# lezhnev74/inverted_index_2

Hardware: NVIDIA B200
Metric: merged postings/s (higher is better)
Workload: dtype u32

## Files before the change

inverted_index_2_b200/csrc/k12_union.cu:

```cuda
#include <algorithm>
#include <cstdlib>
#include <vector>

#include "intcomp.cuh"
#include "keys.cuh"
#include "union.cuh"
#include "union_dev.cuh"

namespace ii2 {

constexpr int K1B_THREADS = 256;
constexpr int K1B_WARPS = K1B_THREADS / 32;
constexpr uint32_t CAP_I = 1024;
constexpr uint32_t K1B_HT = CAP_I > 512 ? 2048 : 1024;
static_assert(CAP_I % K1B_THREADS == 0 && CAP_I <= 1024 && CAP_I % 4 == 0,
              "tile = a whole number of instances per thread, 10-bit tile indexes");
constexpr uint32_t K1B_STAGE_CAP = CAP_I * 6;
constexpr uint32_t K1B_SMALL_D = 64;
constexpr uint32_t K1B_EMPTY = 0xFFFFFFFFu;
constexpr uint32_t K12_PENDING = 0xFFFFFFFFu;
constexpr uint32_t K1B_HEAVY = 0xFFFFFFFFu;

struct K1bArgs {
  const SegDesc* segs;
  int k;
  const uint32_t* part;
  const uint32_t* btb;
  const uint64_t* bpo;
  const uint64_t* bk_pos;
  const uint32_t* bk_cpl;
  const uint64_t* bk_P;
  GroupIn* gin;
  uint32_t* gath;
  uint64_t* src_ptr;
  uint32_t* src_len;
  uint32_t* bk_D;
  uint32_t bucket0;
  const uint32_t* list;
};


__device__ __noinline__ int k1b_tail_compare(const SegDesc* __restrict__ segs, int k, uint32_t ix,
                                             uint32_t nx, uint32_t iy, uint32_t ny, uint32_t skip) {
  int sx, sy;
  uint32_t tx, ty;
  locate_instance(segs, k, ix, sx, tx);
  locate_instance(segs, k, iy, sy, ty);
  const SegDesc& dx = segs[sx];
  const SegDesc& dy = segs[sy];
  const uint32_t ox = __ldg(dx.toff + tx);
  const uint32_t oy = __ldg(dy.toff + ty);
  for (uint32_t c = skip;; c += 16) {
    uint64_t hx, lx, hy, ly;
    load_key16(dx.tb, ox, nx, c, hx, lx);
    load_key16(dy.tb, oy, ny, c, hy, ly);
    if (hx != hy) return hx < hy ? -1 : 1;
    if (lx != ly) return lx < ly ? -1 : 1;
    if (!(nx > c + 16 && ny > c + 16)) break;
  }
  return nx < ny ? -1 : (nx > ny ? 1 : 0);
}

__host__ __device__ inline size_t k1b_smem_bytes(int k) {
  return (size_t)CAP_I * 24
         + (size_t)CAP_I * 4 * 3
         + (size_t)(4 * k) * 4 + (size_t)(2 * k + 2) * 4
         + (size_t)CAP_I * 2 * 2
         + (size_t)k * 40 + 16
         + (size_t)K1B_HT * 4 + 64;
}

constexpr int K1B_MIN_CTAS = 4;
template <bool LIST>
__global__ void __launch_bounds__(K1B_THREADS, K1B_MIN_CTAS) k1b_group_kernel(const K1bArgs a) {
  pdl_enter();
  extern __shared__ __align__(16) uint8_t smem_raw[];
  __shared__ uint64_t s_ws64[K1B_WARPS + 2];
  __shared__ uint32_t s_ws32[K1B_WARPS + 2];
  __shared__ uint32_t s_nreps, s_tot[2];

  const int k = a.k;
  uint8_t* sp = smem_raw;
  uint64_t* key_hi = reinterpret_cast<uint64_t*>(sp); sp += CAP_I * 8;
  uint64_t* key_lo = reinterpret_cast<uint64_t*>(sp); sp += CAP_I * 8;
  uint64_t* key_x = reinterpret_cast<uint64_t*>(sp); sp += CAP_I * 8;
  uint32_t* cg = reinterpret_cast<uint32_t*>(sp); sp += CAP_I * 4;
  uint32_t* inst_a = reinterpret_cast<uint32_t*>(sp); sp += CAP_I * 4;
  uint32_t* pbase = reinterpret_cast<uint32_t*>(sp); sp += CAP_I * 4;
  uint16_t* tlen = reinterpret_cast<uint16_t*>(sp); sp += CAP_I * 2;
  uint16_t* reps = reinterpret_cast<uint16_t*>(sp); sp += CAP_I * 2;
  sp += (16 - (reinterpret_cast<uintptr_t>(sp) & 15)) & 15;
  uint32_t* table = reinterpret_cast<uint32_t*>(sp); sp += K1B_HT * 4;
  uint32_t* cur = reinterpret_cast<uint32_t*>(sp); sp += k * 4;
  uint32_t* mm = reinterpret_cast<uint32_t*>(sp); sp += k * 4;
  uint32_t* hib = reinterpret_cast<uint32_t*>(sp); sp += k * 4;
  uint32_t* endr = reinterpret_cast<uint32_t*>(sp); sp += k * 4;
  uint32_t* rstart = reinterpret_cast<uint32_t*>(sp);
  sp += (2 * k + 2) * 4;
  sp += (8 - (reinterpret_cast<uintptr_t>(sp) & 7)) & 7;
  const uint8_t** sg_tb = reinterpret_cast<const uint8_t**>(sp); sp += k * 8;
  const uint32_t** sg_toff = reinterpret_cast<const uint32_t**>(sp); sp += k * 8;
  const uint64_t** sg_poff = reinterpret_cast<const uint64_t**>(sp); sp += k * 8;
  const uint32_t** sg_post = reinterpret_cast<const uint32_t**>(sp); sp += k * 8;
  uint32_t* sg_bl = reinterpret_cast<uint32_t*>(sp);
  uint32_t* sbase = table;
  uint32_t kp2 = 1;
  while (kp2 < (uint32_t)k) kp2 <<= 1;

  const uint32_t tid = threadIdx.x;
  const unsigned lane = lane_id(), warp = warp_id();
  const uint32_t b = LIST ? a.list[blockIdx.x] : a.bucket0 + blockIdx.x;
  uint32_t W = (uint32_t)(a.bk_pos[b + 1] - a.bk_pos[b]);
  if (W == 0) {
    if (tid == 0) a.bk_D[b] = 0;
    return;
  }
  {
    const uint32_t r0 = b, r1 = b + 1;
    for (int s = tid; s < k; s += K1B_THREADS) {
      cur[s] = a.part[(uint64_t)r0 * k + s];
      endr[s] = a.part[(uint64_t)r1 * k + s];
      const SegDesc sd = a.segs[s];
      sg_tb[s] = sd.tb;
      sg_toff[s] = sd.toff;
      sg_poff[s] = sd.poff;
      sg_post[s] = sd.post;
      sg_bl[s] = sd.base - sd.lo;
      asm volatile("prefetch.global.L2 [%0];" ::"l"(sd.toff + cur[s]));
      asm volatile("prefetch.global.L2 [%0];" ::"l"(sd.poff + cur[s]));
      if (endr[s] - cur[s] > 12) asm volatile("prefetch.global.L2 [%0];" ::"l"(sd.poff + endr[s]));
    }
  }
  const uint64_t rec_base = a.bk_pos[b];
  const uint32_t cpl = a.bk_cpl[b];
  uint32_t* const gath = a.gath + a.bk_P[b];
  uint32_t dcount = 0;
  uint32_t icount = 0;
  uint32_t pcount = 0;
  uint32_t ecount = 0;
  __syncthreads();

  while (W > 0) {
    uint32_t size;
    const uint32_t* mmp;
    if (W <= CAP_I) {
      mmp = endr;
      size = W;
    } else {
      mmp = mm;
      for (int s = tid; s < k; s += K1B_THREADS) hib[s] = endr[s];
      __syncthreads();
      for (;;) {
        uint64_t best = 0;
        for (int s = tid; s < k; s += K1B_THREADS) {
          const uint64_t cand = ((uint64_t)(hib[s] - cur[s]) << 32) | (uint32_t)s;
          best = cand > best ? cand : best;
        }
#pragma unroll
        for (int d = 16; d > 0; d >>= 1) {
          const uint64_t o = __shfl_xor_sync(0xffffffffu, best, d);
          best = o > best ? o : best;
        }
        __syncthreads();
        if (lane == 0) s_ws64[warp] = best;
        __syncthreads();
        for (int w2 = 0; w2 < K1B_WARPS; w2++) best = s_ws64[w2] > best ? s_ws64[w2] : best;
        const int spv = (int)(uint32_t)best;
        const uint32_t win = (uint32_t)(best >> 32);
        const uint32_t mid = cur[spv] + (win >> 1);
        const KeyedTerm pivot = keyed_term(a.segs[spv], mid);
        uint32_t part_sum = 0;
        for (int s = tid; s < k; s += K1B_THREADS) {
          const uint32_t m = s == spv ? mid : keyed_lower_bound(a.segs[s], cur[s], hib[s], pivot);
          mm[s] = m;
          part_sum += m - cur[s];
        }
        uint32_t tot;
        block_exclusive_scan(part_sum, s_ws32, tot);
        size = tot;
        if (size <= CAP_I) break;
        for (int s = tid; s < k; s += K1B_THREADS) hib[s] = mm[s];
        __syncthreads();
      }
      __syncthreads();
    }

    if (k <= 128 && warp != 0) {
    } else if (k <= 128) {
      uint32_t v[4], sum = 0;
#pragma unroll
      for (int j = 0; j < 4; j++) {
        const int s = lane * 4 + j;
        v[j] = s < k ? mmp[s] - cur[s] : 0u;
        sum += v[j];
      }
      uint32_t ex = warp_inclusive_scan(sum) - sum;
#pragma unroll
      for (int j = 0; j < 4; j++) {
        const int s = lane * 4 + j;
        if (s < k) rstart[s] = ex;
        ex += v[j];
      }
      for (uint32_t s2 = k + lane; s2 <= kp2; s2 += 32) rstart[s2] = size;
    } else {
      uint32_t run = 0;
      for (int base = 0; base < k; base += K1B_THREADS) {
        const int s = base + tid;
        const uint32_t v = s < k ? mmp[s] - cur[s] : 0u;
        uint32_t tot;
        const uint32_t ex = block_exclusive_scan(v, s_ws32, tot);
        if (s < k) rstart[s] = run + ex;
        run += tot;
      }
      for (uint32_t s2 = k + tid; s2 <= kp2; s2 += K1B_THREADS) rstart[s2] = size;
    }
    for (uint32_t i = tid; i < K1B_HT / 4; i += K1B_THREADS)
      reinterpret_cast<uint4*>(table)[i] = make_uint4(~0u, ~0u, ~0u, ~0u);
    for (uint32_t i = 4 * tid; i < CAP_I; i += 4 * K1B_THREADS)
      *reinterpret_cast<uint4*>(cg + i) = make_uint4(0u, 0u, 0u, 0u);
    if (tid == 0) s_nreps = 0;
    __syncthreads();

    auto tail_compare = [&](uint32_t x, uint32_t y) -> int {
      const uint32_t skip = cpl + 24;
      const uint32_t nx = tlen[x], ny = tlen[y];
      if (nx > skip && ny > skip)
        return k1b_tail_compare(a.segs, k, inst_a[x], nx, inst_a[y], ny, skip);
      return nx < ny ? -1 : (nx > ny ? 1 : 0);
    };
    auto less = [&](uint16_t x, uint16_t y) -> bool {
      const uint64_t hx = key_hi[x], hy = key_hi[y];
      if (hx != hy) return hx < hy;
      const uint64_t lx = key_lo[x], ly = key_lo[y];
      if (lx != ly) return lx < ly;
      const uint64_t xx = key_x[x], xy = key_x[y];
      if (xx != xy) return xx < xy;
      return tail_compare(x, y) < 0;
    };

    constexpr int PER = CAP_I / K1B_THREADS;
    uint64_t pp[PER];
    uint32_t pl[PER];
    uint32_t og[PER];
    {
      int sg[PER];
      uint32_t ix[PER], to[PER], tn[PER];
      uint64_t p1[PER];
#pragma unroll
      for (int j = 0; j < PER; j++) {
        const uint32_t i = tid + j * K1B_THREADS;
        sg[j] = -1;
        if (i < size) {
          uint32_t lo = 0;
          for (uint32_t step = kp2 >> 1; step > 0; step >>= 1)
            if (rstart[lo + step] <= i) lo += step;
          sg[j] = (int)lo;
          ix[j] = cur[lo] + (i - rstart[lo]);
        }
      }
#pragma unroll
      for (int j = 0; j < PER; j++) {
        if (sg[j] >= 0) {
          const uint32_t* const toff_s = sg_toff[sg[j]];
          const uint64_t* const poff_s = sg_poff[sg[j]];
          to[j] = __ldg(toff_s + ix[j]);
          tn[j] = __ldg(toff_s + ix[j] + 1);
          pp[j] = __ldg(poff_s + ix[j]);
          p1[j] = __ldg(poff_s + ix[j] + 1);
        }
      }
#pragma unroll
      for (int j = 0; j < PER; j++)
        if (sg[j] >= 0) asm volatile("prefetch.global.L2 [%0];" ::"l"(sg_tb[sg[j]] + to[j] + cpl));
#pragma unroll
      for (int j = 0; j < PER; j++) {
        if (sg[j] >= 0) {
          const uint32_t i = tid + j * K1B_THREADS;
          const uint32_t n = tn[j] - to[j];
          uint64_t kh, kl;
          const uint8_t* const tb_s = sg_tb[sg[j]];
          const uint32_t* const post_s = sg_post[sg[j]];
          const uint32_t inst_s = sg_bl[sg[j]] + ix[j];
          load_key16(tb_s, to[j], n, cpl, kh, kl);
          key_hi[i] = kh;
          key_lo[i] = kl;
          key_x[i] = load_key_x(tb_s, to[j], n, cpl);
          tlen[i] = (uint16_t)n;
          inst_a[i] = inst_s;
          pl[j] = (p1[j] - pp[j]) > 0xFFFFFFFEull ? 0xFFFFFFFFu : (uint32_t)(p1[j] - pp[j]);
          pp[j] = reinterpret_cast<uint64_t>(post_s + pp[j]);
          asm volatile("prefetch.global.L2 [%0];" ::"l"(pp[j]));
        }
      }
    }
    __threadfence_block();

#pragma unroll
    for (int j = 0; j < PER; j++) {
      const uint32_t i = tid + j * K1B_THREADS;
      if (i >= size) break;
      const uint64_t kh = key_hi[i], kl = key_lo[i];
      uint32_t h = (uint32_t)kh * 0x9E3779B1u ^ (uint32_t)(kh >> 32) * 0x85EBCA77u ^
                   (uint32_t)kl * 0xC2B2AE3Du ^ (uint32_t)(kl >> 32) * 0x27D4EB2Fu;
      h = (h ^ (h >> 15)) * 0x2C1B3C6Du + tlen[i];
      uint32_t slot = (h ^ (h >> 13)) & (K1B_HT - 1);
      uint32_t rep;
      for (;;) {
        const uint32_t prev = atomicCAS(&table[slot], K1B_EMPTY, i);
        if (prev == K1B_EMPTY) {
          rep = i;
          reps[atomicAdd(&s_nreps, 1u)] = (uint16_t)i;
          break;
        }
        if (*(volatile uint64_t*)&key_hi[prev] == kh && *(volatile uint64_t*)&key_lo[prev] == kl &&
            *(volatile uint16_t*)&tlen[prev] == tlen[i] &&
            *(volatile uint64_t*)&key_x[prev] == key_x[i] && tail_compare(i, prev) == 0) {
          rep = prev;
          break;
        }
        slot = (slot + 1) & (K1B_HT - 1);
      }
      og[j] = (rep << 20) |
              (atomicAdd(&cg[rep], (1u << 20) | (pl[j] > REG_CAP ? REG_CAP + 1 : pl[j])) & 0xFFFFFu);
    }
    __syncthreads();
    const uint32_t D = s_nreps;

    if (D <= K1B_SMALL_D) {
      const unsigned sub = lane & 7u;
#pragma unroll 1
      for (uint32_t t0 = warp * 4; t0 < D; t0 += K1B_WARPS * 4) {
        const uint32_t t = t0 + (lane >> 3);
        const bool valid = t < D;
        const uint32_t me = valid ? reps[t] : 0u;
        uint32_t rank = 0, ib = 0, pst = 0, est = 0;
        if (valid) {
          const uint64_t mh = key_hi[me], ml = key_lo[me], mx = key_x[me];
#pragma unroll 1
          for (uint32_t j = sub; j < D; j += 8) {
            const uint32_t o = reps[j];
            const uint64_t oh = key_hi[o];
            bool lt = oh < mh;
            if (oh == mh && o != me) {
              const uint64_t ol = key_lo[o], ox = key_x[o];
              lt = ol != ml ? ol < ml : (ox != mx ? ox < mx : tail_compare(o, me) < 0);
            }
            const uint32_t c = cg[o];
            const uint32_t len = c & 0xFFFFFu;
            const bool lg = lt && len <= REG_CAP;
            rank += lt ? 1u : 0u;
            ib += lt ? c >> 20 : 0u;
            pst += lg ? len : 0u;
            est += lg ? enc_slot_words(len) : 0u;
          }
        }
#pragma unroll
        for (int d = 4; d > 0; d >>= 1) {
          rank += __shfl_xor_sync(0xffffffffu, rank, d);
          ib += __shfl_xor_sync(0xffffffffu, ib, d);
          pst += __shfl_xor_sync(0xffffffffu, pst, d);
          est += __shfl_xor_sync(0xffffffffu, est, d);
        }
        if (valid && sub == 0) {
          const uint32_t cme = cg[me];
          const uint32_t len = cme & 0xFFFFFu;
          const bool light = len <= REG_CAP;
          const uint32_t src = (uint32_t)rec_base + icount + ib;
          uint4* rec = reinterpret_cast<uint4*>(a.gin + rec_base + dcount + rank);
          rec[0] = make_uint4(inst_a[me], tlen[me], src, cme >> 20);
          rec[1] = make_uint4(len, pcount + pst, ecount + est, 0u);
          sbase[me] = src;
          pbase[me] = light ? pcount + pst : K1B_HEAVY;
          if (rank == D - 1) {
            s_tot[0] = pst + (light ? len : 0u);
            s_tot[1] = est + (light ? enc_slot_words(len) : 0u);
          }
        }
      }
    } else {
      bitonic_sort_any(reps, D, tid, (uint32_t)K1B_THREADS, less, [] { __syncthreads(); });
      __syncthreads();
      uint32_t run_i = 0, run_p = 0, run_e = 0;
      for (uint32_t base = 0; base < D; base += K1B_THREADS) {
        const uint32_t r = base + tid;
        uint32_t me = 0, ci = 0, li = 0, ei = 0;
        uint32_t len = 0;
        if (r < D) {
          me = reps[r];
          ci = cg[me] >> 20;
          len = cg[me] & 0xFFFFFu;
          if (len <= REG_CAP) {
            li = len;
            ei = enc_slot_words(li);
          }
        }
        uint32_t ti, tp, te;
        const uint32_t xi = block_exclusive_scan(ci, s_ws32, ti);
        const uint32_t xp = block_exclusive_scan(li, s_ws32, tp);
        const uint32_t xe = block_exclusive_scan(ei, s_ws32, te);
        if (r < D) {
          GroupIn g;
          g.inst = inst_a[me];
          g.tlen = tlen[me];
          g.src = (uint32_t)rec_base + icount + run_i + xi;
          g.c = ci;
          g.L = len;
          g.pst = pcount + run_p + xp;
          g.eslot = ecount + run_e + xe;
          g.pad = 0;
          a.gin[rec_base + dcount + r] = g;
          sbase[me] = g.src;
          pbase[me] = len <= REG_CAP ? g.pst : K1B_HEAVY;
        }
        run_i += ti;
        run_p += tp;
        run_e += te;
      }
      if (tid == 0) {
        s_tot[0] = run_p;
        s_tot[1] = run_e;
      }
    }
    __syncthreads();

    const uint32_t tile_p = s_tot[0];
    const bool staged = tile_p <= K1B_STAGE_CAP;
    uint32_t* const stage = reinterpret_cast<uint32_t*>(key_hi);
    auto copy_source = [](const uint32_t* __restrict__ src, uint32_t* __restrict__ dst, uint32_t n) {
      uint32_t t = 0;
#pragma unroll 1
      for (; t + 4 <= n; t += 4) {
        const uint32_t x0 = __ldg(src + t), x1 = __ldg(src + t + 1), x2 = __ldg(src + t + 2),
                       x3 = __ldg(src + t + 3);
        dst[t] = x0;
        dst[t + 1] = x1;
        dst[t + 2] = x2;
        dst[t + 3] = x3;
      }
      if (t < n) {
        const uint32_t x0 = __ldg(src + t);
        const uint32_t x1 = t + 1 < n ? __ldg(src + t + 1) : 0u;
        const uint32_t x2 = t + 2 < n ? __ldg(src + t + 2) : 0u;
        dst[t] = x0;
        if (t + 1 < n) dst[t + 1] = x1;
        if (t + 2 < n) dst[t + 2] = x2;
      }
    };
#pragma unroll
    for (int j = 0; j < PER; j++) {
      const uint32_t i = tid + j * K1B_THREADS;
      if (i < size) {
        const uint32_t g = og[j] >> 20;
        const uint32_t pb = pbase[g];
        if (pb != K1B_HEAVY) {
          const uint32_t* src = reinterpret_cast<const uint32_t*>(pp[j]);
          const uint32_t at = pb + (og[j] & 0xFFFFFu);
          if (staged)
            copy_source(src, stage + (at - pcount), pl[j]);
          else
            copy_source(src, gath + at, pl[j]);
        } else {
          const uint32_t at = sbase[g] + ((atomicSub(&cg[g], 1u << 20) >> 20) - 1u);
          a.src_ptr[at] = pp[j];
          a.src_len[at] = pl[j];
        }
      }
    }
    if (staged) {
      __syncthreads();
      uint32_t* const out = gath + pcount;
      const uint32_t head = min(tile_p, (uint32_t)((16u - ((uintptr_t)out & 15u)) & 15u) >> 2);
      if (tid < head) out[tid] = stage[tid];
      const uint32_t nvec = (tile_p - head) >> 2;
      for (uint32_t v = tid; v < nvec; v += K1B_THREADS) {
        const uint32_t e = head + 4 * v;
        *reinterpret_cast<uint4*>(out + e) =
            make_uint4(stage[e], stage[e + 1], stage[e + 2], stage[e + 3]);
      }
      const uint32_t tail0 = head + 4 * nvec;
      if (tail0 + tid < tile_p) out[tail0 + tid] = stage[tail0 + tid];
    }
    dcount += D;
    icount += size;
    pcount += s_tot[0];
    ecount += s_tot[1];
    W -= size;
    if (W == 0) break;
    __syncthreads();
    for (int s = tid; s < k; s += K1B_THREADS) cur[s] = mmp[s];
    __syncthreads();
  }
  if (tid == 0) a.bk_D[b] = dcount;
}


constexpr int K2B_THREADS = 128;
constexpr int K2B_WARPS = K2B_THREADS / 32;
constexpr uint32_t K2B_HALF = 128;
constexpr uint32_t K2B_ENC_WORDS = 3 + 2 * 129 + 1 + (5 * 127 + 3) / 4 + 1;
constexpr uint32_t K2B_EBUF = (K2B_ENC_WORDS + 7) & ~7u;
static_assert(K2B_EBUF / 2 >= 1 + (5 * 127 + 3) / 4, "var-byte stream of 127 values fits a half");

struct K2bArgs {
  const uint64_t* bk_pos;
  const uint64_t* bk_P;
  const uint64_t* bk_E;
  const uint32_t* bk_D;
  const GroupIn* gin;
  RemovedSet rem;
  int want_enc, want_dec, keep_empty;
  GroupRec* recs;
  uint32_t* gath;
  uint32_t* tmp_enc;
  uint64_t* bk_raw;
  uint32_t nb1;
  uint32_t* n_large;
  uint32_t* large_rec;
  uint32_t* large_bucket;
  uint32_t bucket0;
  const uint32_t* list;
};

constexpr int K2B_MIN_CTAS = 8;
template <bool LIST>
__global__ void __launch_bounds__(K2B_THREADS, K2B_MIN_CTAS) k2b_union_kernel(const K2bArgs a) {
  pdl_enter();
  __shared__ __align__(16) uint32_t s_buf[K2B_WARPS][REG_CAP];
  __shared__ __align__(16) uint32_t s_enc[K2B_WARPS][K2B_EBUF];
  const unsigned lane = lane_id(), warp = warp_id();
  const unsigned half = lane >> 4, hl = lane & 15u;
  const uint32_t b = LIST ? a.list[blockIdx.x] : a.bucket0 + blockIdx.x;
  const uint32_t D = a.bk_D[b];
  if (D == 0) return;
  const uint64_t rec_base = a.bk_pos[b];
  uint32_t* const gath = a.gath + a.bk_P[b];
  uint32_t* const enc_base = a.tmp_enc + a.bk_E[b];
  uint32_t acc_t = 0, acc_tb = 0, acc_e = 0;
  uint64_t acc_p = 0;
  const GroupIn g_none = {0u, 0u, 0u, 0u, 0u, 0u, 0u, 0u};
  GroupIn g_next = g_none;
  if (2 * warp + half < D) g_next = a.gin[rec_base + 2 * warp + half];
#pragma unroll 1
  for (uint32_t p0 = 2 * warp; p0 < D; p0 += 2 * K2B_WARPS) {
    const uint32_t r = p0 + half;
    const bool has = r < D;
    const GroupIn g = g_next;
    {
      const uint32_t rn = r + 2 * K2B_WARPS;
      g_next = g_none;
      if (rn < D) g_next = a.gin[rec_base + rn];
    }

    const bool heavy = has && g.L > REG_CAP;
    const bool wide = has && !heavy && g.L >= K2B_HALF;
    if (heavy && hl == 0) {
      const uint32_t slot = atomicAdd(a.n_large, 1u);
      a.large_rec[slot] = (uint32_t)(rec_base + r);
      a.large_bucket[slot] = b;
      GroupRec rec;
      rec.inst = g.inst;
      rec.tlen = g.tlen;
      rec.dec = 0;
      rec.eoff = 0;
      rec.enc = 0;
      rec.cnt = K12_PENDING;
      a.recs[rec_base + r] = rec;
    }
    {
      const bool mine = has && !heavy && !wide;
      const uint32_t L = mine ? g.L : 0u;
      uint32_t* const slot = gath + g.pst;
      uint32_t* const buf = s_buf[warp] + half * K2B_HALF;
      uint32_t* const ebuf = s_enc[warp] + half * (K2B_EBUF / 2);
      const uint32_t outn = union_blocked<16>(slot, buf, L, g.c > 1, a.rem);
      if (a.want_dec)
        for (uint32_t e = hl; e < outn; e += 16) slot[e] = buf[e];
      uint32_t enc = 0;
      uint32_t* const enc_dst = enc_base + g.eslot;
      if (a.want_enc) {
        enc = encode_small_blocked<16>(buf, outn, ebuf);
        for (uint32_t e = hl; e < enc; e += 16) enc_dst[e] = ebuf[e];
      }
      if (mine && hl == 0) {
        GroupRec rec;
        rec.inst = g.inst;
        rec.tlen = g.tlen;
        rec.dec = reinterpret_cast<uint64_t>(slot);
        rec.eoff = a.want_enc ? reinterpret_cast<uint64_t>(enc_dst) : 0ull;
        rec.cnt = outn;
        rec.enc = enc;
        a.recs[rec_base + r] = rec;
        if (outn || a.keep_empty) {
          acc_t += 1;
          acc_tb += g.tlen;
          acc_p += outn;
          acc_e += enc;
        }
      }
      __syncwarp();
    }
    unsigned wmask = __ballot_sync(0xffffffffu, wide && hl == 0);
    while (wmask) {
      const int src = __ffs(wmask) - 1;
      wmask &= wmask - 1;
      GroupIn w;
      w.inst = __shfl_sync(0xffffffffu, g.inst, src);
      w.tlen = __shfl_sync(0xffffffffu, g.tlen, src);
      w.c = __shfl_sync(0xffffffffu, g.c, src);
      w.L = __shfl_sync(0xffffffffu, g.L, src);
      w.pst = __shfl_sync(0xffffffffu, g.pst, src);
      w.eslot = __shfl_sync(0xffffffffu, g.eslot, src);
      const uint32_t rw = p0 + (src >> 4);
      uint32_t* const slot = gath + w.pst;
      uint32_t* const buf = s_buf[warp];
      uint32_t* const ebuf = s_enc[warp];
      const uint32_t outn = union_blocked<32>(slot, buf, w.L, w.c > 1, a.rem);
      if (a.want_dec)
        for (uint32_t e = lane; e < outn; e += 32) slot[e] = buf[e];
      uint32_t enc = 0;
      uint32_t* const enc_dst = enc_base + w.eslot;
      if (a.want_enc && outn) {
        enc = encode_shared_warp(buf, outn, ebuf);
        for (uint32_t e = lane; e < enc; e += 32) enc_dst[e] = ebuf[e];
      }
      if (lane == 0) {
        GroupRec rec;
        rec.inst = w.inst;
        rec.tlen = w.tlen;
        rec.dec = reinterpret_cast<uint64_t>(slot);
        rec.eoff = a.want_enc ? reinterpret_cast<uint64_t>(enc_dst) : 0ull;
        rec.cnt = outn;
        rec.enc = enc;
        a.recs[rec_base + rw] = rec;
        if (outn || a.keep_empty) {
          acc_t += 1;
          acc_tb += w.tlen;
          acc_p += outn;
          acc_e += enc;
        }
      }
      __syncwarp();
    }
  }
  if (hl == 0 && acc_t) {
    unsigned long long* bo = reinterpret_cast<unsigned long long*>(a.bk_raw);
    atomicAdd(&bo[0ull * a.nb1 + b], (unsigned long long)acc_t);
    atomicAdd(&bo[1ull * a.nb1 + b], (unsigned long long)acc_tb);
    atomicAdd(&bo[2ull * a.nb1 + b], (unsigned long long)acc_p);
    atomicAdd(&bo[3ull * a.nb1 + b], (unsigned long long)acc_e);
  }
}

constexpr uint32_t MW_CAP = 1024;
constexpr int MW_V = 32;
constexpr int MW_WARPS = 4;
constexpr int MW_MIN_CTAS = 5;
constexpr uint32_t MW_BUF = MW_CAP + MW_CAP / 32 + 8;
constexpr uint32_t MW_EBUF = 3 + 8 * 129 + 1 + 1 + 6;
static_assert(MW_EBUF >= kMaxSegs + 1, "source prefix fits the stream buffer");

struct MwArgs {
  const uint32_t* n_in_list;
  const uint32_t* in_rec;
  const uint32_t* in_bucket;
  const GroupIn* gin;
  const uint64_t* src_ptr;
  const uint32_t* src_len;
  GroupRec* recs;
  RemovedSet rem;
  int want_enc, keep_empty;
  uint64_t* bk_raw;
  uint32_t nb1;
  uint32_t* cursor;
  uint32_t* n_out_list;
  uint32_t* out_rec;
  uint32_t* out_bucket;
  uint32_t* out_post;
  uint32_t* out_enc;
  unsigned long long* out_cursor;
};

__global__ void __launch_bounds__(MW_WARPS * 32, MW_MIN_CTAS) k2_mwarp_kernel(const MwArgs a) {
  pdl_enter();
  __shared__ __align__(16) uint32_t s_buf[MW_WARPS][MW_BUF];
  __shared__ __align__(16) uint32_t s_enc[MW_WARPS][MW_EBUF];
  const unsigned lane = lane_id(), warp = warp_id();
  uint32_t* const buf = s_buf[warp];
  uint32_t* const ebuf = s_enc[warp];
  uint32_t* const moff = ebuf;
  for (;;) {
    uint32_t item = 0;
    if (lane == 0) item = atomicAdd(a.cursor, 1u);
    item = __shfl_sync(0xffffffffu, item, 0);
    if (item >= *a.n_in_list) return;
    const uint32_t rec = a.in_rec[item], bucket = a.in_bucket[item];
    const GroupIn g = a.gin[rec];
    const uint32_t c = g.c, beg = g.src;
    uint32_t run = 0;
    for (uint32_t base = 0; base < c; base += 32) {
      const uint32_t i = base + lane;
      uint32_t li = i < c ? a.src_len[beg + i] : 0u;
      li = li > MW_CAP + 1 ? MW_CAP + 1 : li;
      const uint32_t inc = warp_inclusive_scan(li);
      if (i < c) moff[i] = min(run + inc - li, MW_CAP + 1);
      run = min(run + __shfl_sync(0xffffffffu, inc, 31), MW_CAP + 1);
    }
    if (run > MW_CAP) {
      if (lane == 0) {
        const uint32_t at = atomicAdd(a.n_out_list, 1u);
        a.out_rec[at] = rec;
        a.out_bucket[at] = bucket;
      }
// ... 699 lines not shown
    const uint32_t ny = std::min<uint32_t>(32768, h_nl - y0);
    uint64_t maxL = 0;
    for (uint32_t i = 0; i < ny; i++) maxL = std::max(maxL, lens[y0 + i]);
    LargeArgs b2 = la;
    b2.rec += y0;
    if (b2.presorted) b2.presorted += y0;
    if (b2.bucket) b2.bucket += y0;
    b2.len += y0;
    b2.off += y0;
    b2.eoff += y0;
    const unsigned gx = (unsigned)std::max<uint64_t>(1, std::min<uint64_t>((maxL + 4095) / 4096, 2048));
    dim3 grid(gx, ny);
    k2_large_gather<<<grid, 256, 0, s>>>(b2, nullptr, 0);
    II2_LAUNCHED();
    uint64_t maxS = 0;
    for (uint32_t i = 0; i < ny; i++) {
      const uint32_t g = y0 + i;
      if (!h_pre[g]) {
        maxS = std::max(maxS, lens[g]);
        continue;
      }
      const uint64_t words = ((uint64_t)h_max[g] >> 5) + 1;
      const uint64_t n_chunks = (words + BM_CHUNK_WORDS - 1) / BM_CHUNK_WORDS;
      II2_CUDA_TRY(cudaMemsetAsync(bm_words.p, 0, words * 4, s));
      k2_large_gather<<<(unsigned)std::min<uint64_t>((lens[g] + 255) / 256, 148 * 16), 256, 0, s>>>(
          b2, bm_words.p, i);
      II2_LAUNCHED();
      k2_bm_count<<<div_up((n_chunks + 1) * 32, 256), 256, 0, s>>>(bm_words.p, words, n_chunks,
                                                                   bm_counts.p, la.rem);
      II2_LAUNCHED();
      II2_TRY(exclusive_scan_u64(bm_counts.p, n_chunks + 1, nullptr, s));
      k2_bm_expand<<<div_up(n_chunks * 32, 256), 256, 0, s>>>(bm_words.p, words, n_chunks,
                                                              bm_counts.p, la.tmp + offs[g],
                                                              d_len.p + g);
      II2_LAUNCHED();
    }
    maxL = maxS;
    k2_large_tile_sort<<<grid, 512, 0, s>>>(b2);
    II2_LAUNCHED();
    for (uint64_t kk = 2ull * LG_TILE; (kk >> 1) < maxL; kk <<= 1) {
      k2_large_stage<<<grid, 256, 0, s>>>(b2, kk, 0);
      II2_LAUNCHED();
      for (uint64_t j = kk >> 2; j >= LG_TILE; j >>= 1) {
        k2_large_stage<<<grid, 256, 0, s>>>(b2, kk, j);
        II2_LAUNCHED();
      }
      k2_large_tile_merge<<<grid, 512, 0, s>>>(b2, kk);
      II2_LAUNCHED();
    }
    k2_large_finish<<<ny, 1024, 0, s>>>(b2);
    II2_LAUNCHED();
  }
  II2_CUDA_TRY(cudaStreamSynchronize(s));
  return II2_OK;
}

static bool k12_takes_fused(uint64_t N, int k) {
  const char* fused_env = getenv("II2_FUSED");
  const bool fused_on = fused_env ? atoi(fused_env) != 0 : N <= 65536;
  return fused_on && k12f_supported(k);
}

int k12_union(const MergePlan& plan, const RemovedSet& rem, bool want_dec, bool want_enc,
              bool keep_empty, uint64_t n_in, uint64_t tb_in, UnionOut& u, cudaStream_t s) {
  u.keep_empty = keep_empty;
  u.want_dec = want_dec;
  u.want_enc = want_enc;
  const uint32_t B = plan.n_buckets, N = plan.n_total;
  const int k = plan.k;
  u.fused = k12_takes_fused(N, k);
  DevBuf<GroupIn> gin;
  DevBuf<uint64_t> src_ptr;
  DevBuf<uint32_t> src_len;
  II2_TRY(gin.alloc_scratch(N, s));
  II2_TRY(src_ptr.alloc_scratch(N, s));
  II2_TRY(src_len.alloc_scratch(N, s));
  II2_TRY(u.recs.alloc_scratch(N, s));
  II2_TRY(u.bk_D.alloc_scratch(B, s));
  II2_TRY(u.bk_raw.alloc_scratch(4 * (size_t)(B + 1), s));
  II2_TRY(u.bk_out.alloc_scratch(4 * (size_t)(B + 1), s));
  II2_TRY(u.totals.alloc_scratch(8, s));
  const uint64_t enc_cap = n_in + n_in / 4 + 6ull * N + 64;
  if (want_enc) II2_TRY(u.tmp_enc.alloc_scratch(enc_cap, s, 16));
  II2_TRY(u.tmp_post.alloc_scratch(n_in, s, 16));
  const uint32_t large_cap = (uint32_t)std::min<uint64_t>(N, n_in / REG_CAP + 1);
  DevBuf<uint32_t> large_u32;
  II2_TRY(large_u32.alloc_scratch(8 * (size_t)large_cap, s));
  DevBuf<unsigned long long> med_cursor;
  II2_TRY(med_cursor.alloc_scratch(8, s));
  II2_CUDA_TRY(cudaMemsetAsync(med_cursor.p, 0, 64, s));
  II2_TRY(u.med_post.alloc_scratch(n_in, s, 16));
  if (want_enc) II2_TRY(u.med_enc.alloc_scratch(n_in + n_in / 4 + 16ull * large_cap + 64, s, 16));
  II2_CUDA_TRY(cudaMemsetAsync(u.totals.p, 0, 64, s));
  II2_CUDA_TRY(cudaMemsetAsync(u.bk_raw.p, 0, 4 * (size_t)(B + 1) * 8, s));
  II2_TRY(u.bk_mode.alloc_scratch(B, s));
  if (u.fused) {
    II2_TRY(u.st_tb.alloc_scratch(tb_in, s, 64));
    II2_TRY(u.st_off.alloc_scratch(3 * (size_t)N, s));
    II2_TRY(u.def_list.alloc_scratch(B, s));
  } else {
    II2_CUDA_TRY(cudaMemsetAsync(u.bk_mode.p, 0, (size_t)B * 4, s));
  }

  K1bArgs a1;
  a1.segs = plan.segs;
  a1.k = k;
  a1.part = plan.part.p;
  a1.btb = plan.btb.p;
  a1.bpo = plan.bpo.p;
  a1.bk_pos = plan.bk_pos();
  a1.bk_cpl = plan.bk_cpl.p;
  a1.bk_P = plan.bk_P();
  a1.gin = gin.p;
  a1.gath = u.tmp_post.p;
  a1.src_ptr = src_ptr.p;
  a1.src_len = src_len.p;
  a1.bk_D = u.bk_D.p;
  K2bArgs a2;
  a2.bk_pos = plan.bk_pos();
  a2.bk_P = plan.bk_P();
  a2.bk_E = plan.bk_E();
  a2.bk_D = u.bk_D.p;
  a2.gin = gin.p;
  a2.rem = rem;
  a2.want_enc = want_enc ? 1 : 0;
  a2.want_dec = want_dec ? 1 : 0;
  a2.keep_empty = keep_empty ? 1 : 0;
  a2.recs = u.recs.p;
  a2.gath = u.tmp_post.p;
  a2.tmp_enc = u.tmp_enc.p;
  a2.bk_raw = u.bk_raw.p;
  a2.nb1 = B + 1;
  a2.n_large = reinterpret_cast<uint32_t*>(u.totals.p + 6);
  a2.large_rec = large_u32.p;
  a2.large_bucket = large_u32.p + large_cap;
  const size_t smem = k1b_smem_bytes(k);
  static size_t attr = 0;
  if (smem > attr) {
    const size_t want = std::max(k1b_smem_bytes(kMaxSegs), smem);
    II2_CUDA_TRY(cudaFuncSetAttribute(k1b_group_kernel<false>, cudaFuncAttributeMaxDynamicSharedMemorySize,
                                      (int)want));
    II2_CUDA_TRY(cudaFuncSetAttribute(k1b_group_kernel<true>, cudaFuncAttributeMaxDynamicSharedMemorySize,
                                      (int)want));
    attr = want;
  }
  auto general = [&](uint32_t grid, const uint32_t* list) -> int {
    a1.bucket0 = a2.bucket0 = 0;
    a1.list = a2.list = list;
    {
      ProfScope scope("k1b_group", s);
      if (list) {
        II2_LAUNCH_CHAIN(k1b_group_kernel<true>, grid, K1B_THREADS, smem, s, a1);
      } else {
        II2_LAUNCH_CHAIN(k1b_group_kernel<false>, grid, K1B_THREADS, smem, s, a1);
      }
    }
    {
      ProfScope scope("k2b_union", s);
      if (list) {
        II2_LAUNCH_CHAIN(k2b_union_kernel<true>, grid, K2B_THREADS, 0, s, a2);
      } else {
        II2_LAUNCH_CHAIN(k2b_union_kernel<false>, grid, K2B_THREADS, 0, s, a2);
      }
    }
    {
      ProfScope scope("k2_medium", s);
      uint32_t* const mid_rec = large_u32.p + 4 * (size_t)large_cap;
      uint32_t* const mid_bucket = large_u32.p + 5 * (size_t)large_cap;
      uint32_t* const n_mid = reinterpret_cast<uint32_t*>(med_cursor.p + 3);
      MwArgs w2;
      w2.n_in_list = a2.n_large;
      w2.in_rec = a2.large_rec;
      w2.in_bucket = a2.large_bucket;
      w2.gin = gin.p;
      w2.src_ptr = src_ptr.p;
      w2.src_len = src_len.p;
      w2.recs = u.recs.p;
      w2.rem = rem;
      w2.want_enc = want_enc ? 1 : 0;
      w2.keep_empty = keep_empty ? 1 : 0;
      w2.bk_raw = u.bk_raw.p;
      w2.nb1 = B + 1;
      w2.cursor = reinterpret_cast<uint32_t*>(med_cursor.p + 2) + 1;
      w2.n_out_list = n_mid;
      w2.out_rec = mid_rec;
      w2.out_bucket = mid_bucket;
      w2.out_post = u.med_post.p;
      w2.out_enc = u.med_enc.p;
      w2.out_cursor = med_cursor.p;
      II2_LAUNCH_CHAIN(k2_mwarp_kernel, kNumSMs * MW_MIN_CTAS, MW_WARPS * 32, 0, s, w2);
      uint32_t* const mid2_rec = large_u32.p + 6 * (size_t)large_cap;
      uint32_t* const mid2_bucket = large_u32.p + 7 * (size_t)large_cap;
      uint32_t* const n_mid2 = reinterpret_cast<uint32_t*>(med_cursor.p + 3) + 1;
      MedArgs m;
      m.n_large = n_mid;
      m.large_rec = mid_rec;
      m.large_bucket = mid_bucket;
      m.gin = gin.p;
      m.src_ptr = src_ptr.p;
      m.src_len = src_len.p;
      m.recs = u.recs.p;
      m.rem = rem;
      m.want_enc = want_enc ? 1 : 0;
      m.keep_empty = keep_empty ? 1 : 0;
      m.bk_raw = u.bk_raw.p;
      m.nb1 = B + 1;
      m.cursor = reinterpret_cast<uint32_t*>(med_cursor.p + 4);
      m.n_huge = n_mid2;
      m.huge_rec = mid2_rec;
      m.huge_bucket = mid2_bucket;
      m.out_post = u.med_post.p;
      m.out_enc = u.med_enc.p;
// ... 92 lines not shown
```

inverted_index_2_b200/csrc/union.cuh:

```cuda
#pragma once
#include "plan.cuh"

namespace ii2 {

struct GroupRec {
  uint64_t dec;
  uint64_t eoff;
  uint32_t inst;
  uint32_t tlen;
  uint32_t cnt;
  uint32_t enc;
};

struct __align__(16) GroupIn {
  uint32_t inst;
  uint32_t tlen;
  uint32_t src;
  uint32_t c;
  uint32_t L;
  uint32_t pst;
  uint32_t eslot;
  uint32_t pad;
};


struct LargeArgs {
  const uint32_t* rec;
  const uint32_t* bucket;
  const GroupIn* gin;
  const uint64_t* src_ptr;
  const uint32_t* src_len;
  uint64_t* len;
  const uint64_t* off;
  const uint64_t* eoff;
  uint32_t* tmp;
  uint32_t* enc;
  GroupRec* recs;
  RemovedSet rem;
  int want_enc, keep_empty;
  int always_sort;
  const uint8_t* presorted;
  uint64_t* bk_raw;
  uint32_t nb1;
};

constexpr uint32_t F_MAXK = 256;
constexpr uint32_t K12F_RECORDS = 0;
constexpr uint32_t K12F_DENSE = 1;
constexpr uint32_t K12F_DEFERRED = 2;

struct K12fArgs {
  const SegDesc* segs;
  int k;
  const uint32_t* part;
  const uint32_t* btb;
  const uint64_t* bpo;
  const uint64_t* bk_pos;
  const uint32_t* bk_cpl;
  const uint64_t* bk_P;
  const uint64_t* bk_E;
  const uint64_t* bk_TB;
  RemovedSet rem;
  int want_enc, want_dec, keep_empty;
  uint32_t* bk_D;
  uint32_t* bk_mode;
  uint64_t* bk_raw;
  uint32_t nb1;
  uint8_t* st_tb;
  uint32_t* st_toff;
  uint32_t* st_eoff;
  uint32_t* st_poff;
  uint32_t* st_enc;
  uint32_t* st_post;
  uint32_t* n_def;
  uint32_t* def_list;
};
bool k12f_supported(int k);
int k12f_launch(const K12fArgs& a, uint32_t n_buckets, cudaStream_t s);

int k2_large_run(LargeArgs la, uint32_t n_groups, DevBuf<uint32_t>& large_tmp,
                 DevBuf<uint32_t>& large_enc, cudaStream_t s);

struct UnionOut {
  DevBuf<GroupRec> recs;
  DevBuf<uint32_t> tmp_post;
  DevBuf<uint32_t> tmp_enc;
  DevBuf<uint32_t> large_enc;
  DevBuf<uint32_t> large_tmp;
  DevBuf<uint32_t> med_post;
  DevBuf<uint32_t> med_enc;
  DevBuf<uint32_t> bk_D;
  bool fused = false;
  DevBuf<uint8_t> st_tb;
  DevBuf<uint32_t> st_off;
  DevBuf<uint32_t> bk_mode;
  DevBuf<uint32_t> def_list;
  uint32_t n_def = 0;
  DevBuf<uint64_t> bk_raw;
  DevBuf<uint64_t> bk_out;
  DevBuf<uint64_t> totals;
  uint64_t h_totals[4] = {0, 0, 0, 0};
  uint64_t terms_merged = 0;
  bool keep_empty = false;
  bool want_dec = false, want_enc = false;
  struct EmitOut* early_out = nullptr;
  bool emitted_early = false;
// ... 27 lines not shown
```

Baseline: 32.66 billion.

## Gather postings in the union kernel via packed source descriptors instead of staging

Stops the grouping kernel from copying every regular group's postings into an intermediate gather buffer. It now writes a compact 64-bit descriptor per source: segment index, first posting offset, clamped length and intra-group offset. The union kernel reads these descriptors and loads postings straight from the segment arrays into shared memory before merging. This is meant to remove a full global write and re-read of all postings, and the decoded output buffer is now allocated only when decoded output is requested. In exchange it adds descriptor packing limits (10-bit segment, 37-bit offset, 9-bit length, 8-bit intra-group offset) and more scattered global loads inside the union kernel.

```diff
diff --git a/inverted_index_2_b200/csrc/k12_union.cu b/inverted_index_2_b200/csrc/k12_union.cu
--- a/inverted_index_2_b200/csrc/k12_union.cu
+++ b/inverted_index_2_b200/csrc/k12_union.cu
@@ -15,7 +15,6 @@
 constexpr uint32_t K1B_HT = CAP_I > 512 ? 2048 : 1024;
 static_assert(CAP_I % K1B_THREADS == 0 && CAP_I <= 1024 && CAP_I % 4 == 0,
               "tile = a whole number of instances per thread, 10-bit tile indexes");
-constexpr uint32_t K1B_STAGE_CAP = CAP_I * 6;
 constexpr uint32_t K1B_SMALL_D = 64;
 constexpr uint32_t K1B_EMPTY = 0xFFFFFFFFu;
 constexpr uint32_t K12_PENDING = 0xFFFFFFFFu;
@@ -29,9 +28,7 @@
   const uint64_t* bpo;
   const uint64_t* bk_pos;
   const uint32_t* bk_cpl;
-  const uint64_t* bk_P;
   GroupIn* gin;
-  uint32_t* gath;
   uint64_t* src_ptr;
   uint32_t* src_len;
   uint32_t* bk_D;
@@ -133,7 +130,6 @@
   }
   const uint64_t rec_base = a.bk_pos[b];
   const uint32_t cpl = a.bk_cpl[b];
-  uint32_t* const gath = a.gath + a.bk_P[b];
   uint32_t dcount = 0;
   uint32_t icount = 0;
   uint32_t pcount = 0;
@@ -239,13 +235,11 @@
     };
 
     constexpr int PER = CAP_I / K1B_THREADS;
-    uint64_t pp[PER];
-    uint32_t pl[PER];
+    uint64_t sd[PER];
     uint32_t og[PER];
     {
       int sg[PER];
       uint32_t ix[PER], to[PER], tn[PER];
-      uint64_t p1[PER];
 #pragma unroll
       for (int j = 0; j < PER; j++) {
         const uint32_t i = tid + j * K1B_THREADS;
@@ -265,8 +259,8 @@
           const uint64_t* const poff_s = sg_poff[sg[j]];
           to[j] = __ldg(toff_s + ix[j]);
           tn[j] = __ldg(toff_s + ix[j] + 1);
-          pp[j] = __ldg(poff_s + ix[j]);
-          p1[j] = __ldg(poff_s + ix[j] + 1);
+          const uint64_t p0 = __ldg(poff_s + ix[j]), np = __ldg(poff_s + ix[j] + 1) - p0;
+          sd[j] = src_desc_pack((uint32_t)sg[j], p0, np > REG_CAP ? REG_CAP + 1 : (uint32_t)np, 0u);
         }
       }
 #pragma unroll
@@ -279,7 +273,6 @@
           const uint32_t n = tn[j] - to[j];
           uint64_t kh, kl;
           const uint8_t* const tb_s = sg_tb[sg[j]];
-          const uint32_t* const post_s = sg_post[sg[j]];
           const uint32_t inst_s = sg_bl[sg[j]] + ix[j];
           load_key16(tb_s, to[j], n, cpl, kh, kl);
           key_hi[i] = kh;
@@ -287,9 +280,6 @@
           key_x[i] = load_key_x(tb_s, to[j], n, cpl);
           tlen[i] = (uint16_t)n;
           inst_a[i] = inst_s;
-          pl[j] = (p1[j] - pp[j]) > 0xFFFFFFFEull ? 0xFFFFFFFFu : (uint32_t)(p1[j] - pp[j]);
-          pp[j] = reinterpret_cast<uint64_t>(post_s + pp[j]);
-          asm volatile("prefetch.global.L2 [%0];" ::"l"(pp[j]));
         }
       }
     }
@@ -320,8 +310,11 @@
         }
         slot = (slot + 1) & (K1B_HT - 1);
       }
-      og[j] = (rep << 20) |
-              (atomicAdd(&cg[rep], (1u << 20) | (pl[j] > REG_CAP ? REG_CAP + 1 : pl[j])) & 0xFFFFFu);
+      uint32_t seg, at, n;
+      uint64_t first;
+      src_desc_unpack(sd[j], seg, first, n, at);
+      atomicAdd(&cg[rep], (1u << 20) | n);
+      og[j] = rep;
     }
     __syncthreads();
     const uint32_t D = s_nreps;
@@ -423,63 +416,32 @@
     }
     __syncthreads();
 
-    const uint32_t tile_p = s_tot[0];
-    const bool staged = tile_p <= K1B_STAGE_CAP;
-    uint32_t* const stage = reinterpret_cast<uint32_t*>(key_hi);
-    auto copy_source = [](const uint32_t* __restrict__ src, uint32_t* __restrict__ dst, uint32_t n) {
-      uint32_t t = 0;
-#pragma unroll 1
-      for (; t + 4 <= n; t += 4) {
-        const uint32_t x0 = __ldg(src + t), x1 = __ldg(src + t + 1), x2 = __ldg(src + t + 2),
-                       x3 = __ldg(src + t + 3);
-        dst[t] = x0;
-        dst[t + 1] = x1;
-        dst[t + 2] = x2;
-        dst[t + 3] = x3;
-      }
-      if (t < n) {
-        const uint32_t x0 = __ldg(src + t);
-        const uint32_t x1 = t + 1 < n ? __ldg(src + t + 1) : 0u;
-        const uint32_t x2 = t + 2 < n ? __ldg(src + t + 2) : 0u;
-        dst[t] = x0;
-        if (t + 1 < n) dst[t + 1] = x1;
-        if (t + 2 < n) dst[t + 2] = x2;
-      }
-    };
+    uint64_t* const stage = key_hi;
+    const uint32_t tile_src = (uint32_t)rec_base + icount;
 #pragma unroll
     for (int j = 0; j < PER; j++) {
       const uint32_t i = tid + j * K1B_THREADS;
       if (i < size) {
-        const uint32_t g = og[j] >> 20;
-        const uint32_t pb = pbase[g];
-        if (pb != K1B_HEAVY) {
-          const uint32_t* src = reinterpret_cast<const uint32_t*>(pp[j]);
-          const uint32_t at = pb + (og[j] & 0xFFFFFu);
-          if (staged)
-            copy_source(src, stage + (at - pcount), pl[j]);
-          else
-            copy_source(src, gath + at, pl[j]);
+        const uint32_t g = og[j];
+        uint32_t seg, at, n;
+        uint64_t first;
+        src_desc_unpack(sd[j], seg, first, n, at);
+        const uint32_t left = atomicSub(&cg[g], (1u << 20) | n);
+        const uint32_t x = sbase[g] + (left >> 20) - 1u - tile_src;
+        if (pbase[g] != K1B_HEAVY) {
+          stage[x] = src_desc_pack(seg, first, n, (left & 0xFFFFFu) - n);
         } else {
-          const uint32_t at = sbase[g] + ((atomicSub(&cg[g], 1u << 20) >> 20) - 1u);
-          a.src_ptr[at] = pp[j];
-          a.src_len[at] = pl[j];
-        }
-      }
-    }
-    if (staged) {
-      __syncthreads();
-      uint32_t* const out = gath + pcount;
-      const uint32_t head = min(tile_p, (uint32_t)((16u - ((uintptr_t)out & 15u)) & 15u) >> 2);
-      if (tid < head) out[tid] = stage[tid];
-      const uint32_t nvec = (tile_p - head) >> 2;
-      for (uint32_t v = tid; v < nvec; v += K1B_THREADS) {
-        const uint32_t e = head + 4 * v;
-        *reinterpret_cast<uint4*>(out + e) =
-            make_uint4(stage[e], stage[e + 1], stage[e + 2], stage[e + 3]);
-      }
-      const uint32_t tail0 = head + 4 * nvec;
-      if (tail0 + tid < tile_p) out[tail0 + tid] = stage[tail0 + tid];
-    }
+          if (n > REG_CAP) {
+            const uint64_t np = __ldg(sg_poff[seg] + cur[seg] + (i - rstart[seg]) + 1) - first;
+            n = np > 0xFFFFFFFEull ? 0xFFFFFFFFu : (uint32_t)np;
+          }
+          stage[x] = reinterpret_cast<uint64_t>(sg_post[seg] + first);
+          a.src_len[tile_src + x] = n;
+        }
+      }
+    }
+    __syncthreads();
+    for (uint32_t v = tid; v < size; v += K1B_THREADS) a.src_ptr[tile_src + v] = stage[v];
     dcount += D;
     icount += size;
     pcount += s_tot[0];
@@ -501,16 +463,60 @@
 constexpr uint32_t K2B_EBUF = (K2B_ENC_WORDS + 7) & ~7u;
 static_assert(K2B_EBUF / 2 >= 1 + (5 * 127 + 3) / 4, "var-byte stream of 127 values fits a half");
 
+template <int W>
+__device__ __forceinline__ void k2b_gather(const SegDesc* __restrict__ segs, const uint64_t* d,
+                                           uint32_t c, uint32_t* buf, unsigned hl) {
+  uint32_t seg, at, n;
+  uint64_t first;
+  if (c == 1) {
+    src_desc_unpack(__ldg(d), seg, first, n, at);
+    const uint32_t* __restrict__ src = segs[seg].post + first;
+    uint32_t x[8];
+#pragma unroll
+    for (int r = 0; r < 8; r++) x[r] = hl + r * W < n ? __ldg(src + hl + r * W) : 0u;
+#pragma unroll
+    for (int r = 0; r < 8; r++)
+      if (hl + r * W < n) buf[hl + r * W] = x[r];
+    return;
+  }
+#pragma unroll 1
+  for (uint32_t j = hl; j < c; j += W) {
+    src_desc_unpack(__ldg(d + j), seg, first, n, at);
+    const uint32_t* __restrict__ src = segs[seg].post + first;
+    uint32_t* const dst = buf + at;
+    uint32_t t = 0;
+#pragma unroll 1
+    for (; t + 4 <= n; t += 4) {
+      const uint32_t x0 = __ldg(src + t), x1 = __ldg(src + t + 1), x2 = __ldg(src + t + 2),
+                     x3 = __ldg(src + t + 3);
+      dst[t] = x0;
+      dst[t + 1] = x1;
+      dst[t + 2] = x2;
+      dst[t + 3] = x3;
+    }
+    if (t < n) {
+      const uint32_t x0 = __ldg(src + t);
+      const uint32_t x1 = t + 1 < n ? __ldg(src + t + 1) : 0u;
+      const uint32_t x2 = t + 2 < n ? __ldg(src + t + 2) : 0u;
+      dst[t] = x0;
+      if (t + 1 < n) dst[t + 1] = x1;
+      if (t + 2 < n) dst[t + 2] = x2;
+    }
+  }
+}
+
 struct K2bArgs {
+  const SegDesc* segs;
   const uint64_t* bk_pos;
   const uint64_t* bk_P;
   const uint64_t* bk_E;
   const uint32_t* bk_D;
   const GroupIn* gin;
+  const uint64_t* src;
   RemovedSet rem;
   int want_enc, want_dec, keep_empty;
   GroupRec* recs;
-  uint32_t* gath;
+  uint32_t* post;
   uint32_t* tmp_enc;
   uint64_t* bk_raw;
   uint32_t nb1;
@@ -533,7 +539,7 @@
   const uint32_t D = a.bk_D[b];
   if (D == 0) return;
   const uint64_t rec_base = a.bk_pos[b];
-  uint32_t* const gath = a.gath + a.bk_P[b];
+  uint32_t* const post = a.post + a.bk_P[b];
   uint32_t* const enc_base = a.tmp_enc + a.bk_E[b];
   uint32_t acc_t = 0, acc_tb = 0, acc_e = 0;
   uint64_t acc_p = 0;
@@ -569,10 +575,12 @@
     {
       const bool mine = has && !heavy && !wide;
       const uint32_t L = mine ? g.L : 0u;
-      uint32_t* const slot = gath + g.pst;
+      uint32_t* const slot = post + g.pst;
       uint32_t* const buf = s_buf[warp] + half * K2B_HALF;
       uint32_t* const ebuf = s_enc[warp] + half * (K2B_EBUF / 2);
-      const uint32_t outn = union_blocked<16>(slot, buf, L, g.c > 1, a.rem);
+      if (mine) k2b_gather<16>(a.segs, a.src + g.src, g.c, buf, hl);
+      __syncwarp();
+      const uint32_t outn = union_blocked<16>(buf, buf, L, g.c > 1, a.rem);
       if (a.want_dec)
         for (uint32_t e = hl; e < outn; e += 16) slot[e] = buf[e];
       uint32_t enc = 0;
@@ -585,7 +593,7 @@
         GroupRec rec;
         rec.inst = g.inst;
         rec.tlen = g.tlen;
-        rec.dec = reinterpret_cast<uint64_t>(slot);
+        rec.dec = a.want_dec ? reinterpret_cast<uint64_t>(slot) : 0ull;
         rec.eoff = a.want_enc ? reinterpret_cast<uint64_t>(enc_dst) : 0ull;
         rec.cnt = outn;
         rec.enc = enc;
@@ -606,15 +614,18 @@
       GroupIn w;
       w.inst = __shfl_sync(0xffffffffu, g.inst, src);
       w.tlen = __shfl_sync(0xffffffffu, g.tlen, src);
+      w.src = __shfl_sync(0xffffffffu, g.src, src);
       w.c = __shfl_sync(0xffffffffu, g.c, src);
       w.L = __shfl_sync(0xffffffffu, g.L, src);
       w.pst = __shfl_sync(0xffffffffu, g.pst, src);
       w.eslot = __shfl_sync(0xffffffffu, g.eslot, src);
       const uint32_t rw = p0 + (src >> 4);
-      uint32_t* const slot = gath + w.pst;
+      uint32_t* const slot = post + w.pst;
       uint32_t* const buf = s_buf[warp];
       uint32_t* const ebuf = s_enc[warp];
-      const uint32_t outn = union_blocked<32>(slot, buf, w.L, w.c > 1, a.rem);
+      k2b_gather<32>(a.segs, a.src + w.src, w.c, buf, lane);
+      __syncwarp();
+      const uint32_t outn = union_blocked<32>(buf, buf, w.L, w.c > 1, a.rem);
       if (a.want_dec)
         for (uint32_t e = lane; e < outn; e += 32) slot[e] = buf[e];
       uint32_t enc = 0;
@@ -627,7 +638,7 @@
         GroupRec rec;
         rec.inst = w.inst;
         rec.tlen = w.tlen;
-        rec.dec = reinterpret_cast<uint64_t>(slot);
+        rec.dec = a.want_dec ? reinterpret_cast<uint64_t>(slot) : 0ull;
         rec.eoff = a.want_enc ? reinterpret_cast<uint64_t>(enc_dst) : 0ull;
         rec.cnt = outn;
         rec.enc = enc;
@@ -1493,7 +1504,7 @@
   II2_TRY(u.totals.alloc_scratch(8, s));
   const uint64_t enc_cap = n_in + n_in / 4 + 6ull * N + 64;
   if (want_enc) II2_TRY(u.tmp_enc.alloc_scratch(enc_cap, s, 16));
-  II2_TRY(u.tmp_post.alloc_scratch(n_in, s, 16));
+  if (want_dec) II2_TRY(u.tmp_post.alloc_scratch(n_in, s, 16));
   const uint32_t large_cap = (uint32_t)std::min<uint64_t>(N, n_in / REG_CAP + 1);
   DevBuf<uint32_t> large_u32;
   II2_TRY(large_u32.alloc_scratch(8 * (size_t)large_cap, s));
@@ -1521,24 +1532,24 @@
   a1.bpo = plan.bpo.p;
   a1.bk_pos = plan.bk_pos();
   a1.bk_cpl = plan.bk_cpl.p;
-  a1.bk_P = plan.bk_P();
   a1.gin = gin.p;
-  a1.gath = u.tmp_post.p;
   a1.src_ptr = src_ptr.p;
   a1.src_len = src_len.p;
   a1.bk_D = u.bk_D.p;
   K2bArgs a2;
+  a2.segs = plan.segs;
   a2.bk_pos = plan.bk_pos();
   a2.bk_P = plan.bk_P();
   a2.bk_E = plan.bk_E();
   a2.bk_D = u.bk_D.p;
   a2.gin = gin.p;
+  a2.src = src_ptr.p;
   a2.rem = rem;
   a2.want_enc = want_enc ? 1 : 0;
   a2.want_dec = want_dec ? 1 : 0;
   a2.keep_empty = keep_empty ? 1 : 0;
   a2.recs = u.recs.p;
-  a2.gath = u.tmp_post.p;
+  a2.post = u.tmp_post.p;
   a2.tmp_enc = u.tmp_enc.p;
   a2.bk_raw = u.bk_raw.p;
   a2.nb1 = B + 1;
diff --git a/inverted_index_2_b200/csrc/union.cuh b/inverted_index_2_b200/csrc/union.cuh
--- a/inverted_index_2_b200/csrc/union.cuh
+++ b/inverted_index_2_b200/csrc/union.cuh
@@ -22,6 +22,18 @@
   uint32_t eslot;
   uint32_t pad;
 };
+
+__host__ __device__ __forceinline__ uint64_t src_desc_pack(uint32_t seg, uint64_t first, uint32_t len,
+                                                           uint32_t at) {
+  return (uint64_t)seg | first << 10 | (uint64_t)len << 47 | (uint64_t)(at & 0xFFu) << 56;
+}
+__host__ __device__ __forceinline__ void src_desc_unpack(uint64_t d, uint32_t& seg, uint64_t& first,
+                                                         uint32_t& len, uint32_t& at) {
+  seg = (uint32_t)d & 0x3FFu;
+  first = (d >> 10) & ((1ull << 37) - 1);
+  len = (uint32_t)(d >> 47) & 0x1FFu;
+  at = (uint32_t)(d >> 56);
+}
 
 
 struct LargeArgs {
```

Result: slower. 31.07 billion (median of 6 runs) (-4.9%).
